# TUMFTM/global_racetrajectory_optimization

Hardware: AMD Instinct MI355X
Metric: min-curv QP solves/sec, N=2000 waypoints, batch=1024 per GPU (higher is better)
Workload: dtype f64

## Files before the change

global_racetrajectory_optimization_amd/csrc/mcq_kernels.hip:

```cpp
#include "mcq_kernels.h"

#include <math.h>



#define MCQ_NT 256
#define MCQ_NW (MCQ_NT / 64)
typedef double d2 __attribute__((vector_size(16)));
typedef __attribute__((address_space(1))) d2 gd2;

#define SM_RED 0
#define SM_S (SM_RED + 64)
#define SPK 1920
#define SM_OVL (SM_S + SPK)
#define OVL_SIZE 7464
#define SM_KV (SM_OVL + OVL_SIZE)
#define SM_KI (SM_KV + 3 * MCQ_KMAX)
#define SM_TOTAL (SM_KI + (3 * MCQ_KMAX + 2 + 1) / 2 + 1)
static_assert(sizeof(double) * SM_TOTAL <= 80 * 1024, "two workgroups of the solver kernel per CU");

size_t mcq_solve_lds_bytes() { return sizeof(double) * SM_TOTAL; }

__shared__ double g_sm[SM_TOTAL];

#ifndef MCQ_IPM_GM_MIN
#define MCQ_IPM_GM_MIN 0.995
#endif
#ifndef MCQ_IPM_GM_C
#define MCQ_IPM_GM_C 10.0
#endif
#ifndef MCQ_TAPIA_RATIO
#define MCQ_TAPIA_RATIO 0.7
#endif
#ifndef MCQ_TAPIA_SHRINK
#define MCQ_TAPIA_SHRINK 0.7
#endif
// ... 441 lines not shown
    }

    gdouble* HD = VEC(w, nm, V_XP);
    gdouble* HU = VEC(w, nm, V_YP);
    for (int i = tid; i < n; i += MCQ_NT) {
        const int ip = i + 1 == n ? 0 : i + 1, im = i == 0 ? n - 1 : i - 1;
        HD[i] = 4.0 * (w.nv[2 * i] * w.nv[2 * i] + w.nv[2 * i + 1] * w.nv[2 * i + 1]);
        HU[i] = -2.0 * (w.nv[2 * i] * w.nv[2 * ip] + w.nv[2 * i + 1] * w.nv[2 * ip + 1]);
        const double px = w.ref[4 * i], py = w.ref[4 * i + 1];
        F[i] = 2.0 * (w.nv[2 * i] * ((px - w.ref[4 * im]) - (w.ref[4 * ip] - px))
                      + w.nv[2 * i + 1] * ((py - w.ref[4 * im + 1]) - (w.ref[4 * ip + 1] - py)));
    }
}


__device__ __noinline__ int factor(const LCtx& c, const gdouble* sig, const gschar* mk, gdouble* fv, bool f32)
{
    if (c.direct) return factor_sp(c, sig, mk);
    c.kkt_f32 = f32 ? 1 : 0;
    if (threadIdx.x == 0) c.f32_count += f32 ? 1 : 0;
    return f32 ? factor_kkt<true>(c, sig, mk, c.kkt_w, fv) : factor_kkt<false>(c, sig, mk, c.kkt_w, fv);
}

__device__ __noinline__ void solve(const LCtx& c, gdouble* v, bool fwd_done)
{
    if (c.direct) { (void)sp_solve(c, v, v); return; }
    if (c.kkt_f32) solve_kkt<true>(c, v, fwd_done);
    else solve_kkt<false>(c, v, fwd_done);
}

__device__ __forceinline__ void apply_Et(const LCtx& c, const gdouble* src, gdouble* dst) { tri_apply_Et(c, src, dst); }

__device__ __noinline__ void gradient(const LCtx& c, const gdouble* x, const gdouble* extra, gdouble* tmp, gdouble* g)
{
    const int n = c.d.n;
    const long long t0 = TICK();
    __syncthreads();
    if (c.direct) {
        const gdouble* HD = VEC(c.w, c.nm, V_SPD);
        const gdouble* HU = VEC(c.w, c.nm, V_SPU);
        const gdouble* F = VEC(c.w, c.nm, V_F);
        for (int i = threadIdx.x; i < n; i += MCQ_NT) {
            const int im = i > 0 ? i - 1 : n - 1, ip = i + 1 < n ? i + 1 : 0;
            g[i] = F[i] + HU[im] * x[im] + HD[i] * x[i] + HU[i] * x[ip];
        }
        __syncthreads();
        if (threadIdx.x == 0) c.tk[2] += TICK() - t0;
        return;
    }
    tri_apply_E(c, x, VEC(c.w, c.nm, V_KREF), MCQ_F_SCALE, tmp);
    if (extra) {
        for (int i = threadIdx.x; i < n; i += MCQ_NT) tmp[i] += extra[i];
        __syncthreads();
    }
    tri_apply_Et(c, tmp, g);
    if (threadIdx.x == 0) c.tk[2] += TICK() - t0;
}

__device__ __forceinline__ int timed_factor(const LCtx& c, const gdouble* sig, const gschar* mk, gdouble* fv = nullptr, bool f32 = false)
{
    const long long t0 = TICK();
    const int r = factor(c, sig, mk, fv, f32);
    if (threadIdx.x == 0) c.tk[0] += TICK() - t0;
    return r;
}
__device__ __forceinline__ void timed_solve(const LCtx& c, gdouble* v, bool fwd_done = false)
{
    const long long t0 = TICK();
    solve(c, v, fwd_done);
    if (threadIdx.x == 0) c.tk[1] += TICK() - t0;
}


__device__ __noinline__ int ipm(const LCtx& c, bool with_kappa)
{
    const int tid = threadIdx.x, n = c.d.n, nm = c.nm;
    double* red = g_sm + SM_RED;
    const gdouble* LO = VEC(c.w, nm, V_LO);
    const gdouble* HI = VEC(c.w, nm, V_HI);
    const gdouble* KR = VEC(c.w, nm, V_KREF);
    gdouble* X = VEC(c.w, nm, V_X);
    gdouble* G = VEC(c.w, nm, V_G);
    gdouble* ZL = VEC(c.w, nm, V_ZL);
    gdouble* ZU = VEC(c.w, nm, V_ZU);
    gdouble* SIG = VEC(c.w, nm, V_SIG);
    gdouble* RHS = VEC(c.w, nm, V_RHS);
    gdouble* DXA = VEC(c.w, nm, V_DXA);
    gdouble* T0 = VEC(c.w, nm, V_T0);
    gdouble* T1 = VEC(c.w, nm, V_T1);
    gdouble* T2 = VEC(c.w, nm, V_T2);
    gdouble* TL = VEC(c.w, nm, V_TL);
    gdouble* TU = VEC(c.w, nm, V_TU);
// ... 350 lines not shown
#define IPB_STORE_X { _Pragma("unroll") for (int u = 0; u < IPB_E; ++u) if (tid + u * MCQ_NT < n) X[tid + u * MCQ_NT] = rx[u]; }
#define IPB_RETURN(v) { rc = (v); goto ipb_flush; }
    unsigned tapia = 0;
    int rc;
#else
#define IPB_STORE_X
#define IPB_RETURN(v) return (v);
#endif

    bool g_exact = true;
    double mu_prev = 1e300;
    int stalled = 0;
#ifndef MCQ_IPM_F32
#define MCQ_IPM_F32 1
#endif
#ifndef MCQ_IPM_F32_RD
#define MCQ_IPM_F32_RD 1e-5
#endif
    bool f32 = MCQ_IPM_F32 && !resume;
#ifndef MCQ_IPM_TRUST_FP64_CARRY
#define MCQ_IPM_TRUST_FP64_CARRY 1
#endif
    bool g_f32 = false;
#if MCQ_IPB_FOLD_P1
    bool folded = false;
    double mu_fold = 0.0, rdm_fold = 0.0;
#endif
    for (int it = 1; it <= c.max_ipm_iter; ++it) {
        double mu;
        for (;;) {
            IPB_PTRS
            double rdm = 0.0;
            mu = 0.0;
#if MCQ_IPB_FOLD_P1
            if (folded) { mu = mu_fold; rdm = rdm_fold; folded = false; }
            else
#endif
            {
#pragma unroll
            for (int h = 0; h < IPB_E / IPB_H; ++h) {
                IPB_HALF(h)
                double x[IPB_H], lo[IPB_H], hi[IPB_H], zl[IPB_H], zu[IPB_H], g[IPB_H];
                int st[IPB_H];
#pragma unroll
                for (int u = 0; u < IPB_H; ++u) {
                    const int i = idx[u];
// ... 32 lines not shown
                    g_exact = true;
                    g_f32 = false;
                    continue;
                }
            }
            if (conv && (g_exact || (MCQ_IPM_TRUST_FP64_CARRY && !resume && !g_f32))) IPB_RETURN(MCQ_OK)
            if (!conv) break;
            IPB_STORE_X
            gradient(c, X, nullptr, VEC(c.w, nm, V_T0), G);
            IPB_RELOAD_G
            g_exact = true;
            g_f32 = false;
        }
        c.out_iters = it;
        if (resume) {
            stalled = mu > 0.9 * mu_prev ? stalled + 1 : 0;
            mu_prev = mu;
            if (stalled >= 3) IPB_RETURN(MCQ_OK)
        }

        const int fs = timed_factor(c, VEC(c.w, c.nm, V_SIG), any_fixed ? c.w.state : nullptr,
                                    VEC(c.w, c.nm, V_RHS), f32);
        if (fs != 0) IPB_RETURN((resume && fs == MCQ_NOT_PD) ? MCQ_OK : fs)
        timed_solve(c, VEC(c.w, c.nm, V_RHS), true);

        double smu;
        {
            IPB_SETUP
            double dxa[IPB_E], sl[IPB_E], su[IPB_E], zl[IPB_E], zu[IPB_E], g[IPB_E];
            bool act[IPB_E];
#pragma unroll
            for (int u = 0; u < IPB_E; ++u) {
                const int i = idx[u];
                act[u] = ok[u] && ST[i] == 0;
#if MCQ_IPB_RESIDENT
                const double x = rx[u];
                dxa[u] = RHS[i]; sl[u] = x - LO[i]; su[u] = HI[i] - x; zl[u] = rl[u]; zu[u] = ru[u]; g[u] = rg[u];
#else
                const double x = X[i];
                dxa[u] = RHS[i]; sl[u] = x - LO[i]; su[u] = HI[i] - x; zl[u] = ZL[i]; zu[u] = ZU[i]; g[u] = G[i];
#endif
            }
            double ap = 1.0, ad = 1.0;
#pragma unroll
            for (int u = 0; u < IPB_E; ++u) {
                if (!ok[u]) continue;
#if MCQ_IPB_NOCOPY
                if (!act[u]) continue;
                const double dx = dxa[u];
#else
                if (!act[u]) { DXA[idx[u]] = 0.0; continue; }
                const double dx = dxa[u];
                DXA[idx[u]] = dx;
#endif
                const double dzla = -zl[u] - zl[u] * dx / sl[u];
                const double dzua = -zu[u] + zu[u] * dx / su[u];
                if (dx < 0.0) ap = fmin(ap, -sl[u] / dx);
                if (dx > 0.0) ap = fmin(ap, su[u] / dx);
                if (dzla < 0.0) ad = fmin(ad, -zl[u] / dzla);
                if (dzua < 0.0) ad = fmin(ad, -zu[u] / dzua);
            }
            block_reduce2_(ap, 1, ad, 1, red);
            double mua = 0.0;
#pragma unroll
            for (int u = 0; u < IPB_E; ++u) {
                if (!act[u]) continue;
                const double dzla = -zl[u] - zl[u] * dxa[u] / sl[u];
                const double dzua = -zu[u] + zu[u] * dxa[u] / su[u];
                mua += (sl[u] + ap * dxa[u]) * (zl[u] + ad * dzla) + (su[u] - ap * dxa[u]) * (zu[u] + ad * dzua);
            }
            mua = block_reduce_(mua, 0, red) / npairs;
            const double ratio = mua / mu;
            smu = ratio * ratio * ratio * mu;
#pragma unroll
            for (int u = 0; u < IPB_E; ++u) {
                if (!ok[u]) continue;
                const double dzla = -zl[u] - zl[u] * dxa[u] / sl[u];
                const double dzua = -zu[u] + zu[u] * dxa[u] / su[u];
                IPB_CORR[idx[u]] = act[u] ? -g[u] + (smu - dxa[u] * dzla) / sl[u] - (smu + dxa[u] * dzua) / su[u] : 0.0;
            }
        }
        timed_solve(c, VEC(c.w, c.nm, MCQ_IPB_NOCOPY ? V_DXA : V_RHS));

        {
            IPB_SETUP
#ifdef MCQ_IPM_FIXED_STEP
            const double gm = 0.995;
#else
            const double gm = fmin(fmax(MCQ_IPM_GM_MIN, 1.0 - MCQ_IPM_GM_C * mu / (zscale * c.wmean)), 1.0 - 1e-9);
#endif
            double amax = 1.0 / gm;
            double dx[IPB_E], da[IPB_E], x[IPB_E], lo[IPB_E], hi[IPB_E], zl[IPB_E], zu[IPB_E], g[IPB_E], sg[IPB_E];
            bool act[IPB_E];
#pragma unroll
            for (int u = 0; u < IPB_E; ++u) {
                const int i = idx[u];
                act[u] = ok[u] && ST[i] == 0;
                dx[u] = IPB_CORR[i]; da[u] = IPB_PRED[i]; lo[u] = LO[i]; hi[u] = HI[i]; sg[u] = SIG[i];
#if MCQ_IPB_RESIDENT
                x[u] = rx[u]; zl[u] = rl[u]; zu[u] = ru[u]; g[u] = rg[u];
#else
                x[u] = X[i]; zl[u] = ZL[i]; zu[u] = ZU[i]; g[u] = G[i];
#endif
            }
#define IPB_STEP3(u)                                                                                                          \
                const double sl = x[u] - lo[u], su = hi[u] - x[u];                                                              \
                const double dzla = -zl[u] - zl[u] * da[u] / sl, dzua = -zu[u] + zu[u] * da[u] / su;                             \
                const double dzl = (-sl * zl[u] + smu - da[u] * dzla - zl[u] * dx[u]) / sl;                                     \
                const double dzu = (-su * zu[u] + smu + da[u] * dzua + zu[u] * dx[u]) / su;
#pragma unroll
            for (int u = 0; u < IPB_E; ++u) {
                if (!act[u]) continue;
                IPB_STEP3(u)
                if (dx[u] < 0.0) amax = fmin(amax, -sl / dx[u]);
                if (dx[u] > 0.0) amax = fmin(amax, su / dx[u]);
                if (dzl < 0.0) amax = fmin(amax, -zl[u] / dzl);
                if (dzu < 0.0) amax = fmin(amax, -zu[u] / dzu);
            }
            amax = block_reduce_(amax, 1, red);
            const double a = fmin(1.0, gm * amax);
            c.last_step = a;
// ... 68 lines not shown
ipb_flush:
    {
        IPB_SETUP
#pragma unroll
        for (int u = 0; u < IPB_E; ++u) {
            if (!ok[u]) continue;
            const int i = idx[u];
            X[i] = rx[u]; ZL[i] = rl[u]; ZU[i] = ru[u]; G[i] = rg[u];
            const unsigned t = (tapia >> (2 * u)) & 3u;
            if (t != 0) IND[i] = (double)((int)t - 2);
        }
    }
    __syncthreads();
    return rc;
#else
    return MCQ_ITER_CAP;
#endif
#undef IPB_SETUP
#undef IPB_RELOAD_G
#undef IPB_STORE_X
#undef IPB_RETURN
#undef IPB_CORR
#undef IPB_PRED
}

struct KappaMem {
    double* kmu;
    double* krh;
    double* mul;
    int* ki;
    int* piv;
    gdouble* sg;
    int cap, ld;
    bool in_lds;
};
__device__ __forceinline__ KappaMem kappa_mem_lds(const LCtx& c)
{
    KappaMem k;
    k.kmu = g_sm + SM_KV;
    k.krh = g_sm + SM_KV + MCQ_KMAX;
    k.mul = g_sm + SM_KV + 2 * MCQ_KMAX;
    k.ki = (int*)(g_sm + SM_KI);
    k.piv = (int*)(g_sm + SM_KI) + 1 + 2 * MCQ_KMAX;
    k.sg = c.w.Z + c.nm;
    k.cap = MCQ_KMAX;
    k.ld = MCQ_KMAX;
// ... 2439 lines not shown
```

global_racetrajectory_optimization_amd/csrc/mcq_kkt.inc:

```
#ifndef MCQ_KKT
#define MCQ_KKT 1
#endif
#ifndef MCQ_KKT_CORR_BATCH
#define MCQ_KKT_CORR_BATCH 1
#endif
#define KKT_CORR_TRIPS_F64 4
#define KKT_CORR_TRIPS_F32 8
#define KKT_FN __device__ __noinline__
#ifndef KKT_TIMERS
#define KKT_TIMERS 0
#endif
#define KT(k) do { if (KKT_TIMERS) { const long long t_ = (long long)wall_clock64(); if (threadIdx.x == 0) c.tk[(k)] += t_ - kt_last; kt_last = t_; } } while (0)
#define KRS 32
#define KCK 8
#define KCKF 16
#define KCK2 6
#define KCOEF 20
#define KAD 20
#define KTRI(r, c) ((r) >= (c) ? (r) * ((r) + 1) / 2 + (c) : (c) * ((c) + 1) / 2 + (r))
#define K_AD(c) ((c).w.L)
#define KAY 26
#define K_OFF(c) ((c).nm >= 64 ? 64 : 0)
#define K_AY(c) ((c).w.L + (size_t)20 * (c).nm + K_OFF(c))
#define KAS 8
#define K_AS(c) ((c).w.L + (size_t)50 * (c).nm + K_OFF(c))
#define K_YV(c) ((c).w.L + (size_t)60 * (c).nm + K_OFF(c))
#define K_TS(c, j) ((c).w.L + (size_t)(66 + (j)) * (c).nm + 64)
static_assert(MCQ_LLD >= 72, "the factor arrays of the saddle-point form (65 doubles per waypoint + 64) and three scratch vectors must fit McqWork.L");
#define KP_SEP 0
#define KP_R0I 160
#define KP_RU0 185
#define KP_RL0 210
#define KP_STEP 240
#define KP_X0 (KP_STEP + 15 * 100)
static_assert(KP_X0 + 160 <= SPK, "separator chain must fit the persistent LDS region");
#define KO_CH 0
#define KO_CH2 (16 * (KCK2 * KAD + 32))
#define KO_AUX (16 * KCK * KRS)
#define KO_RB KO_AUX
#define KO_SPK (KO_AUX + 1280)
#define KO_RR (KO_SPK + 16 * 100)
#define KO_YR (KO_RR + 80)
#define KO_SREC (KO_YR + 80)
#define KO_FLAG (KO_SREC + 16 * KCOEF)
#define KO_TOTAL (KO_FLAG + 8)
#define KS_STRIDE(payload) ((payload) + (8 + 32 - (payload) % 32) % 32)
#define KS_COEF KS_STRIDE(KCKF * KCOEF)
#define KS_CH KS_STRIDE(KCK * KAD)
#define KS_AUX KS_STRIDE(KCK * 8)
#define KS_CH2G KS_STRIDE(KCK2 * KAD)
#define KS_CH2Y KS_STRIDE(KCK2 * 28)
static_assert(KS_COEF % 32 == 8 && KS_CH % 32 == 8 && KS_AUX % 32 == 8 && KS_CH2G % 32 == 8 && KS_CH2Y % 32 == 8, "group strides: 16 banks apart");
#define KS_STG KS_STRIDE(2 * (KAD + KAY))
static_assert(16 * KS_STG <= KO_SREC - KO_SPK && KS_STG % 2 == 0, "staged records of the elimination fit the idle spike / separator regions, 16-byte aligned");
static_assert(16 * KS_AUX <= 1280 && 16 * 75 <= 1280 && 16 * KS_COEF <= 16 * KCK * KRS + 1280 && 16 * KS_CH <= 16 * KCK * KRS
              && 16 * KS_CH2G <= KO_CH2 && KO_CH2 + 16 * KS_CH2Y <= KO_SPK, "overlay regions of the saddle-point elimination");
static_assert(KO_TOTAL <= OVL_SIZE, "scratch of the saddle-point elimination must fit the LDS overlay");

__device__ __forceinline__ double dpp_shl1(double v) { return __builtin_amdgcn_update_dpp(0.0, v, 0x101, 0xf, 0xf, true); }
__device__ __forceinline__ double dpp_shl2(double v) { return __builtin_amdgcn_update_dpp(0.0, v, 0x102, 0xf, 0xf, true); }
__device__ __forceinline__ double dpp_shl5(double v) { return __builtin_amdgcn_update_dpp(0.0, v, 0x105, 0xf, 0xf, true); }
__device__ __forceinline__ double dpp_shl5_low8(double v) { return __builtin_amdgcn_update_dpp(v, v, 0x105, 0xf, 0x3, false); }
__device__ __forceinline__ int kkt_base_index(int c, int r, bool first)
{
    if (r == 0) return c == 0 ? 0 : c == 3 ? 1 : c == 4 ? 2 : c == 8 ? 15 : c == 9 ? 16 : c == 15 ? 17 : (first && c == 13) ? 7 : (first && c == 14) ? 8 : 18;
    if (r == 1) return c == 1 ? 3 : c == 2 ? 4 : c == 3 ? 6 : c == 8 ? 19 : (first && c == 13) ? 9 : 18;
// ... 89 lines not shown
    KktRaw r;
    kkt_point_load(c, sig, mk, wgt, fv, m, r);
    kkt_point_make(r, rec);
    if (c.chain) kkt_chain_ends(rec, m, c.d.n);
}

#define KKT_LO_APPLY(lo, s, t)                                                                                 \
    do {                                                                                                       \
        t[0] = lo[0] * s[3] + lo[1] * s[4];                                                                    \
        t[1] = lo[2] * s[3];                                                                                   \
        t[2] = lo[2] * s[4];                                                                                   \
        t[3] = fma(lo[3], s[0], s[1]);                                                                         \
        t[4] = fma(lo[4], s[0], s[2]);                                                                         \
    } while (0)
#define KKT_UP_APPLY(up, s, t)                                                                                 \
    do {                                                                                                       \
        t[0] = up[3] * s[3] + up[4] * s[4];                                                                    \
        t[1] = s[3];                                                                                           \
        t[2] = s[4];                                                                                           \
        t[3] = up[0] * s[0] + up[2] * s[1];                                                                    \
        t[4] = up[1] * s[0] + up[2] * s[2];                                                                    \
    } while (0)

template <int K> __device__ __forceinline__ void kkt_gj_stage(double (&v)[5], int c, bool& bad)
{
    constexpr int RHO = K == 0 ? 3 : K == 1 ? 4 : K == 2 ? 1 : K == 3 ? 2 : 0;
    constexpr int GAM = K == 0 ? 1 : K == 1 ? 2 : K == 2 ? 3 : K == 3 ? 4 : 0;
    const double piv = bcast_row16<GAM>(v[RHO]);
#ifdef IPM_TRACE
    if ((threadIdx.x & 15) == 0 && !(fabs(piv) > 1e-6) ) printf("   gj stage %d pivot %.3e (tid %d)\n", K, piv, (int)threadIdx.x);
#endif
    bad |= !(fabs(piv) > 1e-290);
    const double inv = kkt_rcp(piv);
    const bool own = (c == GAM);
    const double keep = own ? 0.0 : 1.0;
    const double vk = own ? 1.0 : v[RHO];
    const double pr = vk * inv;
#pragma unroll
    for (int j = 0; j < 5; ++j) {
        if (j == RHO) continue;
        v[j] = fnma_bcast_row16<GAM>(v[j], pr, v[j] * keep);
    }
    v[RHO] = pr;
}
__device__ __forceinline__ void kkt_gj(double (&v)[5], int c, bool& bad)
{
// ... 65 lines not shown
    const int nseg = G.nseg, Lmax = G.Lmax;
    double* per = g_sm + SM_S;
    double* ovl = g_sm + SM_OVL;
    const bool has = g < nseg;
    const int s0 = has ? KSEP(g, n, nseg) : 0;
    const int s1 = has ? (g + 1 < nseg ? KSEP(g + 1, n, nseg) : n) : 1;
    const int lo_pt = s0 + 1, L = s1 - s0 - 1;
    RG* AD = (RG*)K_AD(c);
    RG* AS = (RG*)K_AS(c);
    RG* AY = (RG*)K_AY(c);
    const bool chain = c.chain != 0;
    bool bad = false;
    long long kt_last = KKT_TIMERS ? (long long)wall_clock64() : 0;

    __syncthreads();
    if (tid == 0) ovl[KO_FLAG] = 0.0;
    if (tid < nseg) {
        double rec[KCOEF];
        kkt_point_record(c, sig, mk, wgt, nullptr, KSEP(tid, n, nseg), rec);
#pragma unroll
        for (int q = 0; q < KCOEF; ++q) ovl[KO_SREC + tid * KCOEF + q] = rec[q];
#pragma unroll
        for (int q = 0; q < 10; ++q) per[KP_SEP + tid * 10 + q] = rec[7 + q];
    }

    double v[5] = {0.0, 0.0, 0.0, 0.0, 0.0};
    double* coef = ovl + KO_CH + g * KS_COEF;
    int ixF[5], ixN[5];
#pragma unroll
    for (int r = 0; r < 5; ++r) { ixF[r] = kkt_base_index(cl, r, true); ixN[r] = kkt_base_index(cl, r, false); }
    const int colp = kkt_col_of_lane(cl);
    RG* const st_base = cl < 5 ? AD : cl < 15 ? AY + (cl - 11) : AY + 20;
    const int st_rec = cl < 5 ? KAD : KAYR;
    int st_off[5];
    bool st_en[5];
#pragma unroll
    for (int r = 0; r < 5; ++r) {
        st_off[r] = cl < 5 ? KTRI(r, colp) : cl < 15 ? r * 4 : r;
        st_en[r] = cl < 5 ? r >= colp : (cl >= 11 && cl < 15) || (cl == 15 && fv != nullptr);
    }
    constexpr int PER = KRec<F32>::PER;
    constexpr int STG_SLOT = KAD + KAYR;
    constexpr int NI_AD = KAD / PER, NI_AY = KAYR / PER;
    constexpr int NJ = (2 * (NI_AD + NI_AY) + 15) / 16;
    static_assert(KAD % PER == 0 && KAYR % PER == 0 && 2 * STG_SLOT * sizeof(RT) <= KS_STG * sizeof(double), "staged records: whole items, inside the group's slice");
    RT* const stg = (RT*)(ovl + KO_SPK + g * KS_STG);
// ... 97 lines not shown
#pragma unroll
                for (int r = 0; r < 5; ++r) spk[75 + r * 5 + (cl - 5)] = v[r];
            } else if (cl >= 10 && cl < 15) {
                if (cl > 10) AS[(size_t)m * KAS + (cl - 11)] = (RT)v[0];
#pragma unroll
                for (int r = 0; r < 5; ++r) spk[50 + r * 5 + (cl - 10)] = v[r];
            } else if (cl == 15 && fv) {
                fv[m] = v[0];
#pragma unroll
                for (int r = 0; r < 5; ++r) per[KP_X0 + g * 10 + 5 + r] = v[r];
            }
        }
        RG* const sp_rec = cl >= 10 ? AS + (cl - 11) : AS + 4 + (cl - 6);
        const bool sp_on = (cl > 5 && cl < 10) || (cl > 10 && cl < 15) || (cl == 15 && fv != nullptr);
        double* chG = ovl + KO_CH + g * KS_CH2G;
        double* chY = ovl + KO_CH2 + g * KS_CH2Y;
        const int nq = (Lmax - 1 + KCK2 - 1) / KCK2;
        double up_prev[5] = {0.0, 0.0, 0.0, 0.0, 0.0};
        if (has) {
#pragma unroll
            for (int r = 0; r < 5; ++r) up_prev[r] = (double)AD[(size_t)(lo_pt + L - 1) * KAD + 15 + r];
        }
        const double l3f = has ? (double)AD[(size_t)lo_pt * KAD + 18] : 0.0, l4f = has ? (double)AD[(size_t)lo_pt * KAD + 19] : 0.0;
        KItem rg[(KCK2 * KAD / KRec<F32>::PER + 15) / 16], ry[(KCK2 * KAYR / KRec<F32>::PER + 15) / 16];
        if (nq > 0) {
            kkt_stage_issue<F32, KCK2 * KAD>(AD + (size_t)(lo_pt + (nq - 1) * KCK2) * KAD, cl, rg);
            kkt_stage_issue<F32, KCK2 * KAYR>(AY + (size_t)(lo_pt + (nq - 1) * KCK2) * KAYR, cl, ry);
        }
        for (int q = nq - 1; q >= 0; --q) {
            __builtin_amdgcn_wave_barrier();
            kkt_stage_commit<F32, KCK2 * KAD>(chG, cl, rg);
            kkt_stage_commit<F32, KCK2 * KAYR>(chY, cl, ry);
            __builtin_amdgcn_wave_barrier();
            if (q > 0) {
                kkt_stage_issue<F32, KCK2 * KAD>(AD + (size_t)(lo_pt + (q - 1) * KCK2) * KAD, cl, rg);
                kkt_stage_issue<F32, KCK2 * KAYR>(AY + (size_t)(lo_pt + (q - 1) * KCK2) * KAYR, cl, ry);
            }
            const int cy4 = cl >= 11 && cl < 15 ? cl - 11 : 0;
#define KKT_YREAD(b_, r_) ((b_)[cl == 15 ? 20 + (r_) : (r_) * 4 + cy4])
            double g_c[15], y_c[5], lo_c[5];
#pragma unroll
            for (int e = 0; e < 15; ++e) g_c[e] = chG[(KCK2 - 1) * KAD + e];
#pragma unroll
            for (int r = 0; r < 5; ++r) { y_c[r] = KKT_YREAD(chY + (KCK2 - 1) * KAYR, r); lo_c[r] = chG[(KCK2 - 1) * KAD + 15 + r]; }
#pragma unroll
            for (int kk = KCK2 - 1; kk >= 0; --kk) {
// ... 210 lines not shown
            const int e = tid + q * MCQ_NT;
            m_[q] = 0.0;
            if (e < (nseg - 1) * 25) {
                const double* ps = per + KP_STEP + (e / 25) * 100;
                const int r = (e % 25) / 5, cc = e % 5;
#pragma unroll
                for (int j = 0; j < 5; ++j) m_[q] = fma(ps[r * 5 + j], ps[50 + j * 5 + cc], m_[q]);
            }
        }
        __syncthreads();
#pragma unroll
        for (int q = 0; q < 2; ++q) {
            const int e = tid + q * MCQ_NT;
            if (e < (nseg - 1) * 25) per[KP_STEP + (e / 25) * 100 + 50 + e % 25] = m_[q];
        }
    }
    KT(2);
    const bool fail = ovl[KO_FLAG] != 0.0;
    __syncthreads();
    return fail ? MCQ_NOT_PD : 0;
}

template <bool F32>
KKT_FN void solve_kkt(const LCtx& c, gdouble* vv, bool fwd_done)
{
    typedef typename KRec<F32>::G RG;
    typedef typename KRec<F32>::T RT;
    const int tid = threadIdx.x, lane = tid & 63, wv = tid >> 6;
    const int cl = lane & 15, g = 4 * wv + (lane >> 4);
    const int n = c.d.n;
    const KktGeom G = kkt_geom(n);
    const int nseg = G.nseg, Lmax = G.Lmax;
    double* per = g_sm + SM_S;
    double* ovl = g_sm + SM_OVL;
    const bool has = g < nseg;
    const int s0 = has ? KSEP(g, n, nseg) : 0;
    const int s1 = has ? (g + 1 < nseg ? KSEP(g + 1, n, nseg) : n) : 1;
    const int lo_pt = s0 + 1, L = s1 - s0 - 1;
    const RG* AD = (const RG*)K_AD(c);
    const RG* AS = (const RG*)K_AS(c);
    RG* YV = (RG*)K_YV(c);
    double* ch = ovl + KO_CH + g * KS_CH;
    double* aux = ovl + KO_AUX + g * KS_AUX;
    const int rr_ = cl < 5 ? cl : 4;
    int ro[5];
#pragma unroll
    for (int j = 0; j < 5; ++j) ro[j] = KTRI(rr_, j);
    const int nq = (Lmax + KCK - 1) / KCK;
    long long kt_last = KKT_TIMERS ? (long long)wall_clock64() : 0;
    __syncthreads();

    if (!fwd_done) {
        KItem rg[(KCK * KAD / KRec<F32>::PER + 15) / 16];
        double rv;
        kkt_stage_issue<F32, KCK * KAD>(AD + (size_t)lo_pt * KAD, cl, rg);
        { int m = lo_pt + cl; m = m < n ? m : n - 1; rv = vv[m]; }
        double y = 0.0;
        for (int q = 0; q < nq; ++q) {
            __builtin_amdgcn_wave_barrier();
            kkt_stage_commit<F32, KCK * KAD>(ch, cl, rg);
            aux[cl] = rv;
            __builtin_amdgcn_wave_barrier();
            if (q + 1 < nq) {
                kkt_stage_issue<F32, KCK * KAD>(AD + (size_t)(lo_pt + (q + 1) * KCK) * KAD, cl, rg);
                int m = lo_pt + (q + 1) * KCK + cl; m = m < n ? m : n - 1; rv = vv[m];
            }
            double lo_c[5], dr_c[5], rk_c;
#pragma unroll
            for (int j = 0; j < 5; ++j) { lo_c[j] = ch[15 + j]; dr_c[j] = ch[ro[j]]; }
            rk_c = aux[0];
#pragma unroll
            for (int kk = 0; kk < KCK; ++kk) {
                const int k = q * KCK + kk;
// ... 2 lines not shown
                if (kk + 1 < KCK) {
                    const double* rn = ch + (kk + 1) * KAD;
#pragma unroll
                    for (int j = 0; j < 5; ++j) { lo_n[j] = rn[15 + j]; dr_n[j] = rn[ro[j]]; }
                    rk_n = aux[kk + 1];
                }
                double yb[5], t[5];
                yb[0] = bcast_row16<0>(y); yb[1] = bcast_row16<1>(y); yb[2] = bcast_row16<2>(y); yb[3] = bcast_row16<3>(y); yb[4] = bcast_row16<4>(y);
                KKT_LO_APPLY(lo_c, yb, t);
                t[0] = rk_c - t[0];
                const double yn = (dr_c[0] * t[0] - dr_c[1] * t[1]) - (dr_c[2] * t[2] + dr_c[3] * t[3]) - dr_c[4] * t[4];
                if (active) {
                    y = yn;
                    if (cl < 5) YV[(size_t)(lo_pt + k) * 5 + cl] = (RT)yn;
                }
                if (kk + 1 < KCK) {
#pragma unroll
                    for (int j = 0; j < 5; ++j) { lo_c[j] = lo_n[j]; dr_c[j] = dr_n[j]; }
                    rk_c = rk_n;
                }
            }
        }
    }
    __syncthreads();
    KT(3);

    if (!fwd_done) {
#define KKT_Y_ISSUE(qq)                                                                                              \
    _Pragma("unroll") for (int i = 0; i < (KCK * 5 + 15) / 16; ++i) {                                                \
        const int e = cl + 16 * i;                                                                                   \
        int m = lo_pt + (qq) * KCK + e / 5;                                                                          \
        m = m < n ? m : n - 1;                                                                                       \
        ry[i] = (double)YV[(size_t)m * 5 + e % 5];                                                                         \
    }
        KItem rg[(KCK * KAD / KRec<F32>::PER + 15) / 16];
        double ry[(KCK * 5 + 15) / 16];
        kkt_stage_issue<F32, KCK * KAD>(AD + (size_t)(lo_pt + (nq - 1) * KCK) * KAD, cl, rg);
        KKT_Y_ISSUE(nq - 1)
        double x = 0.0;
        double up_prev[5] = {0.0, 0.0, 0.0, 0.0, 0.0};
        double* x0s = per + KP_X0 + g * 10;
        for (int q = nq - 1; q >= 0; --q) {
            __builtin_amdgcn_wave_barrier();
            kkt_stage_commit<F32, KCK * KAD>(ch, cl, rg);
#pragma unroll
            for (int i = 0; i < (KCK * 5 + 15) / 16; ++i)
// ... 20 lines not shown
                double xb[5], t[5];
                xb[0] = bcast_row16<0>(x); xb[1] = bcast_row16<1>(x); xb[2] = bcast_row16<2>(x); xb[3] = bcast_row16<3>(x); xb[4] = bcast_row16<4>(x);
                KKT_UP_APPLY(up_prev, xb, t);
                const double xn = yk_c - ((gr_c[0] * t[0] + gr_c[1] * t[1]) + (gr_c[2] * t[2] + gr_c[3] * t[3]) + gr_c[4] * t[4]);
                if (active) {
                    x = xn;
#pragma unroll
                    for (int j = 0; j < 5; ++j) up_prev[j] = lo_c[j];
                    const int m = lo_pt + k;
                    if (cl == 0) vv[m] = xn;
                    if (cl < 5) {
                        if (k == L - 1) x0s[5 + cl] = xn;
                        if (k == 0) x0s[cl] = xn;
                    }
                }
                if (kk > 0) {
#pragma unroll
                    for (int j = 0; j < 5; ++j) { gr_c[j] = gr_n[j]; lo_c[j] = lo_n[j]; }
                    yk_c = yk_n;
                }
            }
        }
    }
    __syncthreads();
    KT(4);

    if (wv == 0) {
        double* rr = ovl + KO_RR;
        double* yr = ovl + KO_YR;
        if (lane < nseg) {
            const int j = lane, jp = j > 0 ? j - 1 : nseg - 1;
            const double* sp = per + KP_SEP + j * 10;
            const double lo[5] = {sp[0], sp[1], sp[2], sp[3], sp[4]};
            const double up[5] = {sp[5], sp[6], sp[7], sp[8], sp[9]};
            double xf[5], xl[5], t[5], u[5];
#pragma unroll
            for (int q = 0; q < 5; ++q) { xf[q] = per[KP_X0 + j * 10 + q]; xl[q] = per[KP_X0 + jp * 10 + 5 + q]; }
            if (c.chain && j == 0) {
#pragma unroll
                for (int q = 0; q < 5; ++q) xl[q] = 0.0;
            }
            KKT_UP_APPLY(up, xf, u);
            KKT_LO_APPLY(lo, xl, t);
            rr[j * 5 + 0] = vv[KSEP(j, n, nseg)] - u[0] - t[0];
#pragma unroll
            for (int q = 1; q < 5; ++q) rr[j * 5 + q] = -u[q] - t[q];
        }
        __builtin_amdgcn_wave_barrier();
        const double* r0i = per + KP_R0I + rr_ * 5;
        if (nseg == 1) {
            const double x0 = (r0i[0] * rr[0] + r0i[1] * rr[1]) + (r0i[2] * rr[2] + r0i[3] * rr[3]) + r0i[4] * rr[4];
            __builtin_amdgcn_wave_barrier();
            if (lane < 5) rr[lane] = x0;
        } else {
            const int LR = nseg - 1;
#pragma unroll
            for (int q = 0; q < 2; ++q) {
                const int e = lane + 64 * q;
                if (e < LR * 5) {
                    const double* dr = per + KP_STEP + (e / 5) * 100 + (e % 5) * 5;
                    const double* rk = rr + (e / 5 + 1) * 5;
                    yr[e] = (dr[0] * rk[0] + dr[1] * rk[1]) + (dr[2] * rk[2] + dr[3] * rk[3]) + dr[4] * rk[4];
                }
            }
            __builtin_amdgcn_wave_barrier();
            double y = 0.0;
            for (int k = 0; k < LR; ++k) {
// ... 18 lines not shown
            __builtin_amdgcn_wave_barrier();
            double r0[5];
#pragma unroll
            for (int r = 0; r < 5; ++r) {
                double acc = rr[r];
#pragma unroll
                for (int j = 0; j < 5; ++j) acc -= per[KP_RU0 + r * 5 + j] * yr[j] + per[KP_RL0 + r * 5 + j] * yr[(LR - 1) * 5 + j];
                r0[r] = acc;
            }
            const double x0 = (r0i[0] * r0[0] + r0i[1] * r0[1]) + (r0i[2] * r0[2] + r0i[3] * r0[3]) + r0i[4] * r0[4];
            double x0b[5];
            x0b[0] = bcast_row16<0>(x0); x0b[1] = bcast_row16<1>(x0); x0b[2] = bcast_row16<2>(x0); x0b[3] = bcast_row16<3>(x0); x0b[4] = bcast_row16<4>(x0);
            __builtin_amdgcn_wave_barrier();
            if (lane < 5) rr[lane] = x0;
#pragma unroll
            for (int q = 0; q < 2; ++q) {
                const int e = lane + 64 * q;
                if (e < LR * 5) {
                    const double* xs = per + KP_STEP + (e / 5) * 100 + 75 + (e % 5) * 5;
                    rr[5 + e] = yr[e] - ((xs[0] * x0b[0] + xs[1] * x0b[1]) + (xs[2] * x0b[2] + xs[3] * x0b[3]) + xs[4] * x0b[4]);
                }
            }
        }
    }
    __syncthreads();
    KT(5);

    if (has) {
        const double* rr = ovl + KO_RR;
        const int gn = g + 1 < nseg ? g + 1 : 0;
        double xa[5], xb[5];
#pragma unroll
        for (int q = 0; q < 5; ++q) { xa[q] = rr[g * 5 + q]; xb[q] = rr[gn * 5 + q]; }
#ifdef MCQ_PERTURB_ULP
        for (int q = 0; q < 5; ++q) { xa[q] *= 1.0 + 0x1p-52; xb[q] *= 1.0 + 0x1p-52; }
#endif
        if (cl == 0) vv[s0] = xa[0];
        if (L > 0) {
            const RG* adf = (const RG*)K_AD(c) + (size_t)lo_pt * KAD;
            const double* sr = per + KP_SEP + gn * 10;
            xa[1] = fma((double)adf[18], xa[0], xa[1]);
            xa[2] = fma((double)adf[19], xa[0], xa[2]);
            if (!(c.chain && gn == 0)) {
                xb[1] = fma(sr[0] / sr[2], xb[0], xb[1]);
                xb[2] = fma(sr[1] / sr[2], xb[0], xb[2]);
            }
        }
#if MCQ_KKT_CORR_BATCH
        constexpr int KKT_CB = F32 ? KKT_CORR_TRIPS_F32 : KKT_CORR_TRIPS_F64;
        for (int k0 = cl; k0 < L; k0 += 16 * KKT_CB) {
            int idx[KKT_CB];
            bool ok[KKT_CB];
#pragma unroll
            for (int u = 0; u < KKT_CB; ++u) {
                ok[u] = k0 + 16 * u < L;
                idx[u] = lo_pt + (ok[u] ? k0 + 16 * u : k0);
            }
            RT as[KKT_CB][KAS];
            double acc[KKT_CB];
#pragma unroll
            for (int u = 0; u < KKT_CB; ++u) {
                const RG* src = AS + (size_t)idx[u] * KAS;
#pragma unroll
                for (int q = 0; q < KAS; ++q) as[u][q] = src[q];
                acc[u] = vv[idx[u]];
            }
#pragma unroll
            for (int u = 0; u < KKT_CB; ++u) {
#pragma unroll
                for (int q = 0; q < 4; ++q) acc[u] -= (double)as[u][q] * xa[1 + q] + (double)as[u][4 + q] * xb[1 + q];
            }
#pragma unroll
            for (int u = 0; u < KKT_CB; ++u)
                if (ok[u]) vv[idx[u]] = acc[u];
        }
#else
        for (int k = cl; k < L; k += 16) {
            const int m = lo_pt + k;
            const RG* as = AS + (size_t)m * KAS;
            double acc = vv[m];
#pragma unroll
            for (int q = 0; q < 4; ++q) acc -= (double)as[q] * xa[1 + q] + (double)as[4 + q] * xb[1 + q];
            vv[m] = acc;
        }
#endif
    }
    __syncthreads();
    KT(6);
}
```

Baseline: 104,500.

## Defer KKT back-substitution correction into IPM consumers via LDS separator table

Instead of having solve_kkt run its final back-substitution correction pass over all points and write them to global memory, the solve now stores, per segment, the folded separator values in an LDS table and returns early. The IPM predictor and corrector loops then rebuild each needed solution entry on the fly from that table, the AS coefficients and the partial vector. It also precomputes the fold coefficients into persistent LDS, which removes the per-solve divisions and global loads, and drops two barriers when the forward pass is already done. The aim is to cut a full global read-modify-write sweep plus a block barrier on each solve. In exchange, consumers pay for a segment lookup and extra AS loads per entry, and the persistent LDS region grows.

```diff
diff --git a/global_racetrajectory_optimization_amd/csrc/mcq_kernels.hip b/global_racetrajectory_optimization_amd/csrc/mcq_kernels.hip
--- a/global_racetrajectory_optimization_amd/csrc/mcq_kernels.hip
+++ b/global_racetrajectory_optimization_amd/csrc/mcq_kernels.hip
@@ -11,7 +11,7 @@
 
 #define SM_RED 0
 #define SM_S (SM_RED + 64)
-#define SPK 1920
+#define SPK 1964
 #define SM_OVL (SM_S + SPK)
 #define OVL_SIZE 7464
 #define SM_KV (SM_OVL + OVL_SIZE)
@@ -499,11 +499,11 @@
     return f32 ? factor_kkt<true>(c, sig, mk, c.kkt_w, fv) : factor_kkt<false>(c, sig, mk, c.kkt_w, fv);
 }
 
-__device__ __noinline__ void solve(const LCtx& c, gdouble* v, bool fwd_done)
+__device__ __noinline__ void solve(const LCtx& c, gdouble* v, bool fwd_done, bool defer)
 {
     if (c.direct) { (void)sp_solve(c, v, v); return; }
-    if (c.kkt_f32) solve_kkt<true>(c, v, fwd_done);
-    else solve_kkt<false>(c, v, fwd_done);
+    if (c.kkt_f32) solve_kkt<true>(c, v, fwd_done, defer);
+    else solve_kkt<false>(c, v, fwd_done, defer);
 }
 
 __device__ __forceinline__ void apply_Et(const LCtx& c, const gdouble* src, gdouble* dst) { tri_apply_Et(c, src, dst); }
@@ -541,10 +541,10 @@
     if (threadIdx.x == 0) c.tk[0] += TICK() - t0;
     return r;
 }
-__device__ __forceinline__ void timed_solve(const LCtx& c, gdouble* v, bool fwd_done = false)
+__device__ __forceinline__ void timed_solve(const LCtx& c, gdouble* v, bool fwd_done = false, bool defer = false)
 {
     const long long t0 = TICK();
-    solve(c, v, fwd_done);
+    solve(c, v, fwd_done, defer);
     if (threadIdx.x == 0) c.tk[1] += TICK() - t0;
 }
 
@@ -941,6 +941,19 @@
 #define MCQ_IPM_TRUST_FP64_CARRY 1
 #endif
     bool g_f32 = false;
+#if MCQ_IPB_DEFER_CORR
+    const bool defer = !c.direct;
+#define IPB_SOLUTION(VV, OUT)                                                                                          \
+    if (!defer) {                                                                                                      \
+        _Pragma("unroll") for (int u = 0; u < IPB_E; ++u) OUT[u] = VV[idx[u]];                                         \
+    } else if (c.kkt_f32) kkt_deferred_entries<true, IPB_E>(c, VV, idx, OUT);                                          \
+    else {                                                                                                             \
+        _Pragma("unroll") for (int h = 0; h < IPB_E / KKT_CORR_TRIPS_F64; ++h)                                         \
+            kkt_deferred_entries<false, KKT_CORR_TRIPS_F64>(c, VV, idx + h * KKT_CORR_TRIPS_F64, OUT + h * KKT_CORR_TRIPS_F64); \
+    }
+#else
+    const bool defer = false;
+#endif
 #if MCQ_IPB_FOLD_P1
     bool folded = false;
     double mu_fold = 0.0, rdm_fold = 0.0;
@@ -1019,25 +1032,39 @@
         const int fs = timed_factor(c, VEC(c.w, c.nm, V_SIG), any_fixed ? c.w.state : nullptr,
                                     VEC(c.w, c.nm, V_RHS), f32);
         if (fs != 0) IPB_RETURN((resume && fs == MCQ_NOT_PD) ? MCQ_OK : fs)
-        timed_solve(c, VEC(c.w, c.nm, V_RHS), true);
+        timed_solve(c, VEC(c.w, c.nm, V_RHS), true, defer);
 
         double smu;
         {
             IPB_SETUP
             double dxa[IPB_E], sl[IPB_E], su[IPB_E], zl[IPB_E], zu[IPB_E], g[IPB_E];
             bool act[IPB_E];
+#if MCQ_IPB_DEFER_CORR
+#define IPB_DXA_LOAD(u, i)
+#else
+#define IPB_DXA_LOAD(u, i) dxa[u] = RHS[i];
+#endif
 #pragma unroll
             for (int u = 0; u < IPB_E; ++u) {
                 const int i = idx[u];
                 act[u] = ok[u] && ST[i] == 0;
 #if MCQ_IPB_RESIDENT
                 const double x = rx[u];
-                dxa[u] = RHS[i]; sl[u] = x - LO[i]; su[u] = HI[i] - x; zl[u] = rl[u]; zu[u] = ru[u]; g[u] = rg[u];
+                IPB_DXA_LOAD(u, i) sl[u] = x - LO[i]; su[u] = HI[i] - x; zl[u] = rl[u]; zu[u] = ru[u]; g[u] = rg[u];
 #else
                 const double x = X[i];
-                dxa[u] = RHS[i]; sl[u] = x - LO[i]; su[u] = HI[i] - x; zl[u] = ZL[i]; zu[u] = ZU[i]; g[u] = G[i];
-#endif
-            }
+                IPB_DXA_LOAD(u, i) sl[u] = x - LO[i]; su[u] = HI[i] - x; zl[u] = ZL[i]; zu[u] = ZU[i]; g[u] = G[i];
+#endif
+            }
+#undef IPB_DXA_LOAD
+#if MCQ_IPB_DEFER_CORR
+            IPB_SOLUTION(RHS, dxa)
+#if MCQ_IPB_NOCOPY
+#pragma unroll
+            for (int u = 0; u < IPB_E; ++u)
+                if (defer && ok[u]) IPB_PRED[idx[u]] = dxa[u];
+#endif
+#endif
             double ap = 1.0, ad = 1.0;
 #pragma unroll
             for (int u = 0; u < IPB_E; ++u) {
@@ -1077,7 +1104,7 @@
                 IPB_CORR[idx[u]] = act[u] ? -g[u] + (smu - dxa[u] * dzla) / sl[u] - (smu + dxa[u] * dzua) / su[u] : 0.0;
             }
         }
-        timed_solve(c, VEC(c.w, c.nm, MCQ_IPB_NOCOPY ? V_DXA : V_RHS));
+        timed_solve(c, VEC(c.w, c.nm, MCQ_IPB_NOCOPY ? V_DXA : V_RHS), false, defer);
 
         {
             IPB_SETUP
@@ -1089,11 +1116,17 @@
             double amax = 1.0 / gm;
             double dx[IPB_E], da[IPB_E], x[IPB_E], lo[IPB_E], hi[IPB_E], zl[IPB_E], zu[IPB_E], g[IPB_E], sg[IPB_E];
             bool act[IPB_E];
+#if MCQ_IPB_DEFER_CORR
+            IPB_SOLUTION(IPB_CORR, dx)
+#endif
 #pragma unroll
             for (int u = 0; u < IPB_E; ++u) {
                 const int i = idx[u];
                 act[u] = ok[u] && ST[i] == 0;
-                dx[u] = IPB_CORR[i]; da[u] = IPB_PRED[i]; lo[u] = LO[i]; hi[u] = HI[i]; sg[u] = SIG[i];
+#if !MCQ_IPB_DEFER_CORR
+                dx[u] = IPB_CORR[i];
+#endif
+                da[u] = IPB_PRED[i]; lo[u] = LO[i]; hi[u] = HI[i]; sg[u] = SIG[i];
 #if MCQ_IPB_RESIDENT
                 x[u] = rx[u]; zl[u] = rl[u]; zu[u] = ru[u]; g[u] = rg[u];
 #else
@@ -1208,6 +1241,7 @@
 #undef IPB_RETURN
 #undef IPB_CORR
 #undef IPB_PRED
+#undef IPB_SOLUTION
 }
 
 struct KappaMem {
diff --git a/global_racetrajectory_optimization_amd/csrc/mcq_kkt.inc b/global_racetrajectory_optimization_amd/csrc/mcq_kkt.inc
--- a/global_racetrajectory_optimization_amd/csrc/mcq_kkt.inc
+++ b/global_racetrajectory_optimization_amd/csrc/mcq_kkt.inc
@@ -6,6 +6,9 @@
 #endif
 #define KKT_CORR_TRIPS_F64 4
 #define KKT_CORR_TRIPS_F32 8
+#ifndef MCQ_IPB_DEFER_CORR
+#define MCQ_IPB_DEFER_CORR 1
+#endif
 #define KKT_FN __device__ __noinline__
 #ifndef KKT_TIMERS
 #define KKT_TIMERS 0
@@ -33,7 +36,8 @@
 #define KP_RL0 210
 #define KP_STEP 240
 #define KP_X0 (KP_STEP + 15 * 100)
-static_assert(KP_X0 + 160 <= SPK, "separator chain must fit the persistent LDS region");
+#define KP_FOLD (KP_X0 + 160)
+static_assert(KP_FOLD + 64 <= SPK, "separator chain must fit the persistent LDS region");
 #define KO_CH 0
 #define KO_CH2 (16 * (KCK2 * KAD + 32))
 #define KO_AUX (16 * KCK * KRS)
@@ -42,6 +46,9 @@
 #define KO_RR (KO_SPK + 16 * 100)
 #define KO_YR (KO_RR + 80)
 #define KO_SREC (KO_YR + 80)
+#define KO_TAB KO_SREC
+#define KTAB 10
+static_assert(KTAB <= KCOEF && KTAB % 2 == 0, "the correction's table inside the separators' records, entries 16-byte aligned");
 #define KO_FLAG (KO_SREC + 16 * KCOEF)
 #define KO_TOTAL (KO_FLAG + 8)
 #define KS_STRIDE(payload) ((payload) + (8 + 32 - (payload) % 32) % 32)
@@ -177,6 +184,22 @@
         t[4] = up[1] * s[0] + up[2] * s[2];                                                                    \
     } while (0)
 
+template <typename RT> __device__ __forceinline__ double kkt_corr_value(const double* te, bool sep, double v, const RT (&as)[KAS])
+{
+    double acc = v;
+#pragma unroll
+    for (int q = 0; q < 4; ++q) acc -= (double)as[q] * te[q] + (double)as[4 + q] * te[4 + q];
+    return sep ? te[8] : acc;
+}
+__device__ __forceinline__ int kkt_corr_segment(const double* tab, int i, float seg_per_point, int nseg)
+{
+    int j = (int)((float)i * seg_per_point);
+    j = j < nseg - 1 ? j : nseg - 1;
+    if ((double)i < tab[j * KTAB + 9]) --j;
+    else if (j + 1 < nseg && (double)i >= tab[(j + 1) * KTAB + 9]) ++j;
+    return j;
+}
+
 template <int K> __device__ __forceinline__ void kkt_gj_stage(double (&v)[5], int c, bool& bad)
 {
     constexpr int RHO = K == 0 ? 3 : K == 1 ? 4 : K == 2 ? 1 : K == 3 ? 2 : 0;
@@ -288,6 +311,10 @@
         for (int q = 0; q < KCOEF; ++q) ovl[KO_SREC + tid * KCOEF + q] = rec[q];
 #pragma unroll
         for (int q = 0; q < 10; ++q) per[KP_SEP + tid * 10 + q] = rec[7 + q];
+        const int gl = tid > 0 ? tid - 1 : nseg - 1;
+        const bool fold = !(chain && tid == 0);
+        per[KP_FOLD + gl * 4 + 2] = fold ? rec[7] / rec[9] : 0.0;
+        per[KP_FOLD + gl * 4 + 3] = fold ? rec[8] / rec[9] : 0.0;
     }
 
     double v[5] = {0.0, 0.0, 0.0, 0.0, 0.0};
@@ -431,6 +458,7 @@
             for (int r = 0; r < 5; ++r) up_prev[r] = (double)AD[(size_t)(lo_pt + L - 1) * KAD + 15 + r];
         }
         const double l3f = has ? (double)AD[(size_t)lo_pt * KAD + 18] : 0.0, l4f = has ? (double)AD[(size_t)lo_pt * KAD + 19] : 0.0;
+        if (has && cl == 0) { per[KP_FOLD + g * 4] = l3f; per[KP_FOLD + g * 4 + 1] = l4f; }
         KItem rg[(KCK2 * KAD / KRec<F32>::PER + 15) / 16], ry[(KCK2 * KAYR / KRec<F32>::PER + 15) / 16];
         if (nq > 0) {
             kkt_stage_issue<F32, KCK2 * KAD>(AD + (size_t)(lo_pt + (nq - 1) * KCK2) * KAD, cl, rg);
@@ -687,7 +715,7 @@
 }
 
 template <bool F32>
-KKT_FN void solve_kkt(const LCtx& c, gdouble* vv, bool fwd_done)
+KKT_FN void solve_kkt(const LCtx& c, gdouble* vv, bool fwd_done, bool defer)
 {
     typedef typename KRec<F32>::G RG;
     typedef typename KRec<F32>::T RT;
@@ -714,6 +742,10 @@
     const int nq = (Lmax + KCK - 1) / KCK;
     long long kt_last = KKT_TIMERS ? (long long)wall_clock64() : 0;
     __syncthreads();
+#if MCQ_IPB_DEFER_CORR
+    double vsep = 0.0;
+    if (wv == 0 && lane < nseg) vsep = vv[KSEP(lane, n, nseg)];
+#endif
 
     if (!fwd_done) {
         KItem rg[(KCK * KAD / KRec<F32>::PER + 15) / 16];
@@ -762,6 +794,9 @@
             }
         }
     }
+#if MCQ_IPB_DEFER_CORR
+    if (!fwd_done)
+#endif
     __syncthreads();
     KT(3);
 
@@ -828,6 +863,9 @@
             }
         }
     }
+#if MCQ_IPB_DEFER_CORR
+    if (!fwd_done)
+#endif
     __syncthreads();
     KT(4);
 
@@ -848,7 +886,11 @@
             }
             KKT_UP_APPLY(up, xf, u);
             KKT_LO_APPLY(lo, xl, t);
+#if MCQ_IPB_DEFER_CORR
+            rr[j * 5 + 0] = vsep - u[0] - t[0];
+#else
             rr[j * 5 + 0] = vv[KSEP(j, n, nseg)] - u[0] - t[0];
+#endif
 #pragma unroll
             for (int q = 1; q < 5; ++q) rr[j * 5 + q] = -u[q] - t[q];
         }
@@ -913,30 +955,41 @@
                 }
             }
         }
+#if MCQ_IPB_DEFER_CORR
+        __builtin_amdgcn_wave_barrier();
+        if (lane < nseg) {
+            const int j = lane, gn = j + 1 < nseg ? j + 1 : 0;
+            double xa[5], xb[5];
+#pragma unroll
+            for (int q = 0; q < 5; ++q) { xa[q] = rr[j * 5 + q]; xb[q] = rr[gn * 5 + q]; }
+#ifdef MCQ_PERTURB_ULP
+            for (int q = 0; q < 5; ++q) { xa[q] *= 1.0 + 0x1p-52; xb[q] *= 1.0 + 0x1p-52; }
+#endif
+            const double* fc = per + KP_FOLD + j * 4;
+            xa[1] = fma(fc[0], xa[0], xa[1]);
+            xa[2] = fma(fc[1], xa[0], xa[2]);
+            if (!(c.chain && gn == 0)) {
+                xb[1] = fma(fc[2], xb[0], xb[1]);
+                xb[2] = fma(fc[3], xb[0], xb[2]);
+            }
+            double* te = ovl + KO_TAB + j * KTAB;
+#pragma unroll
+            for (int q = 0; q < 4; ++q) { te[q] = xa[1 + q]; te[4 + q] = xb[1 + q]; }
+            te[8] = xa[0];
+            te[9] = (double)KSEP(j, n, nseg);
+        }
+#endif
     }
     __syncthreads();
     KT(5);
 
+#if MCQ_IPB_DEFER_CORR
+    if (defer) return;
     if (has) {
-        const double* rr = ovl + KO_RR;
-        const int gn = g + 1 < nseg ? g + 1 : 0;
-        double xa[5], xb[5];
-#pragma unroll
-        for (int q = 0; q < 5; ++q) { xa[q] = rr[g * 5 + q]; xb[q] = rr[gn * 5 + q]; }
-#ifdef MCQ_PERTURB_ULP
-        for (int q = 0; q < 5; ++q) { xa[q] *= 1.0 + 0x1p-52; xb[q] *= 1.0 + 0x1p-52; }
-#endif
-        if (cl == 0) vv[s0] = xa[0];
-        if (L > 0) {
-            const RG* adf = (const RG*)K_AD(c) + (size_t)lo_pt * KAD;
-            const double* sr = per + KP_SEP + gn * 10;
-            xa[1] = fma((double)adf[18], xa[0], xa[1]);
-            xa[2] = fma((double)adf[19], xa[0], xa[2]);
-            if (!(c.chain && gn == 0)) {
-                xb[1] = fma(sr[0] / sr[2], xb[0], xb[1]);
-                xb[2] = fma(sr[1] / sr[2], xb[0], xb[2]);
-            }
-        }
+        double x[9];
+#pragma unroll
+        for (int q = 0; q < 9; ++q) x[q] = ovl[KO_TAB + g * KTAB + q];
+        if (cl == 0) vv[s0] = x[8];
 #if MCQ_KKT_CORR_BATCH
         constexpr int KKT_CB = F32 ? KKT_CORR_TRIPS_F32 : KKT_CORR_TRIPS_F64;
         for (int k0 = cl; k0 < L; k0 += 16 * KKT_CB) {
@@ -957,6 +1010,62 @@
                 acc[u] = vv[idx[u]];
             }
 #pragma unroll
+            for (int u = 0; u < KKT_CB; ++u) acc[u] = kkt_corr_value<RT>(x, false, acc[u], as[u]);
+#pragma unroll
+            for (int u = 0; u < KKT_CB; ++u)
+                if (ok[u]) vv[idx[u]] = acc[u];
+        }
+#else
+        for (int k = cl; k < L; k += 16) {
+            const int m = lo_pt + k;
+            RT as[KAS];
+#pragma unroll
+            for (int q = 0; q < KAS; ++q) as[q] = AS[(size_t)m * KAS + q];
+            vv[m] = kkt_corr_value<RT>(x, false, vv[m], as);
+        }
+#endif
+    }
+#else
+    (void)defer;
+    if (has) {
+        const double* rr = ovl + KO_RR;
+        const int gn = g + 1 < nseg ? g + 1 : 0;
+        double xa[5], xb[5];
+#pragma unroll
+        for (int q = 0; q < 5; ++q) { xa[q] = rr[g * 5 + q]; xb[q] = rr[gn * 5 + q]; }
+#ifdef MCQ_PERTURB_ULP
+        for (int q = 0; q < 5; ++q) { xa[q] *= 1.0 + 0x1p-52; xb[q] *= 1.0 + 0x1p-52; }
+#endif
+        if (cl == 0) vv[s0] = xa[0];
+        if (L > 0) {
+            const double* fc = per + KP_FOLD + g * 4;
+            xa[1] = fma(fc[0], xa[0], xa[1]);
+            xa[2] = fma(fc[1], xa[0], xa[2]);
+            if (!(c.chain && gn == 0)) {
+                xb[1] = fma(fc[2], xb[0], xb[1]);
+                xb[2] = fma(fc[3], xb[0], xb[2]);
+            }
+        }
+#if MCQ_KKT_CORR_BATCH
+        constexpr int KKT_CB = F32 ? KKT_CORR_TRIPS_F32 : KKT_CORR_TRIPS_F64;
+        for (int k0 = cl; k0 < L; k0 += 16 * KKT_CB) {
+            int idx[KKT_CB];
+            bool ok[KKT_CB];
+#pragma unroll
+            for (int u = 0; u < KKT_CB; ++u) {
+                ok[u] = k0 + 16 * u < L;
+                idx[u] = lo_pt + (ok[u] ? k0 + 16 * u : k0);
+            }
+            RT as[KKT_CB][KAS];
+            double acc[KKT_CB];
+#pragma unroll
+            for (int u = 0; u < KKT_CB; ++u) {
+                const RG* src = AS + (size_t)idx[u] * KAS;
+#pragma unroll
+                for (int q = 0; q < KAS; ++q) as[u][q] = src[q];
+                acc[u] = vv[idx[u]];
+            }
+#pragma unroll
             for (int u = 0; u < KKT_CB; ++u) {
 #pragma unroll
                 for (int q = 0; q < 4; ++q) acc[u] -= (double)as[u][q] * xa[1 + q] + (double)as[u][4 + q] * xb[1 + q];
@@ -976,6 +1085,35 @@
         }
 #endif
     }
+#endif
     __syncthreads();
     KT(6);
 }
+
+#if MCQ_IPB_DEFER_CORR
+template <bool F32, int NE>
+__device__ __forceinline__ void kkt_deferred_entries(const LCtx& c, const gdouble* vv, const int* idx, double* out)
+{
+    typedef typename KRec<F32>::G RG;
+    typedef typename KRec<F32>::T RT;
+    const int n = c.d.n, nseg = kkt_geom(n).nseg;
+    const double* tab = g_sm + SM_OVL + KO_TAB;
+    const RG* AS = (const RG*)K_AS(c);
+    const float seg_per_point = (float)nseg / (float)n;
+    RT as[NE][KAS];
+    double v[NE];
+#pragma unroll
+    for (int u = 0; u < NE; ++u) {
+        const RG* src = AS + (size_t)idx[u] * KAS;
+#pragma unroll
+        for (int q = 0; q < KAS; ++q) as[u][q] = src[q];
+        v[u] = vv[idx[u]];
+    }
+#pragma unroll
+    for (int u = 0; u < NE; ++u) {
+        const int j = kkt_corr_segment(tab, idx[u], seg_per_point, nseg);
+        const double* te = tab + j * KTAB;
+        out[u] = kkt_corr_value<RT>(te, (double)idx[u] == te[9], v[u], as[u]);
+    }
+}
+#endif
```

Result: no change. 104,700 (median of 6 runs) (+0.2%).
